# pierluigiferrari/ssd_keras

Hardware: AMD Instinct MI355X
Metric: images/sec SSD300 fwd+decode @batch32 (higher is better)
Workload: dtype f32 (decode, threshold, TF-style f32 NMS, top-k); bf16 conv backbone; 1 GPU; SSD300 VGG-16 inference (mode='inference': forward + DecodeDetections), 21 classes, batch 32 per GPU, conf 0.01 / NMS 0.45 / top-200, random-init weights, synthetic 300x300x3 uint8-range images; per_gpu_batch=32, global_batch=32, conv_dtype=bf16, parallelism=replicas x1, launch=hip_graph (forward + DecodeDetections captured once, replayed per step), decode_stream=same stream; DecodeDetections reads the head outputs directly (no y_pred in HBM)

## Files before the change

### ssd_keras_amd/csrc/ssdhip_decode.hip

```cpp
#include <hip/hip_runtime.h>
#include <stdint.h>
#include <stdlib.h>

#include "ssdhip.h"
#include "ssdhip_math.h"
#include "ssdhip_tile.h"
#include "ssdhip_heads.h"
#include "ssdhip_decode64.h"

#ifdef SSDHIP_PROFILE
__device__ unsigned long long g_prof[64];
#define PROF_DECL long long _pt = clock64(); long long _pa[12] = {0, 0, 0, 0, 0, 0, 0, 0, 0, 0, 0, 0};
#define PROF_MARK(i) { const long long _t = clock64(); _pa[i] += _t - _pt; _pt = _t; }
#define PROF_FLUSH(base) if (threadIdx.x == 0) { for (int _i = 0; _i < 12; ++_i) if (_pa[_i]) atomicAdd(&g_prof[(base) + _i], (unsigned long long)_pa[_i]); }
extern "C" int ssdhip_profile_read(unsigned long long* host_out, int reset) {
    if (hipMemcpyFromSymbol(host_out, HIP_SYMBOL(g_prof), sizeof(g_prof)) != hipSuccess) return -1;
    if (reset) { unsigned long long z[64] = {0}; if (hipMemcpyToSymbol(HIP_SYMBOL(g_prof), z, sizeof(z)) != hipSuccess) return -1; }
    return 0;
}
#else
#define PROF_DECL
#define PROF_MARK(i)
#define PROF_FLUSH(base)
#endif

namespace ssdhip {

constexpr int IDX_BITS = 20;
constexpr u32 IDX_MASK = (1u << IDX_BITS) - 1u;
constexpr int DIGIT_BITS = 13;
constexpr int NBINS = 1 << DIGIT_BITS;
constexpr int NMS_BIN_SHIFT = 14;
constexpr int NMS_NBINS = 4096;
#ifndef SSDHIP_MAX_CHUNK
#define SSDHIP_MAX_CHUNK 512
#endif
#ifndef SSDHIP_NMS_MINWAVES
#define SSDHIP_NMS_MINWAVES 3
#endif
constexpr int MAX_CHUNK = SSDHIP_MAX_CHUNK;
constexpr int KEPT_LDS = 256;
constexpr int KC_KEYS = 9216;
constexpr int TOPK_SORT_MAX = 4096;

struct DecodeParams {
    int B, N, C, L, G;
    int class_agnostic, semantics, coords, border;
    int thr_inclusive;
    float thr_eff;
    u32 thr_key;
    int iou_f32;
    int fast_ok;
    int px_f32;
    int no_nms;
    float filter_kE;
    double iou_thresh, img_w, img_h;
    int top_k, cap, cap_store, out_rows, sorted;
    int no_dma;
};

template <int SHIFT, int NB>
__device__ __forceinline__ int bin_of(u32 skey, u32 thr_key) {
    const u32 v = skey >> SHIFT, base = thr_key >> SHIFT;
    if (v <= base) return 0;
    const u32 d = v - base;
    return d > (u32)(NB - 1) ? NB - 1 : (int)d;
}

template <int SEM>
__device__ __forceinline__ float decode_center(float off, float var, float a_wh, float a_c) {
    if (SEM == SSDHIP_SEM_KERAS) return (off * var) * a_wh + a_c;
    if (SEM == SSDHIP_SEM_DEBUG) return (off * a_wh) * var + a_c;
    return off * (var * a_wh) + a_c;
}

__device__ __forceinline__ void scan_tile_body(const float* tile, int* wave_cnt, const DecodeParams& p, const int b, const int a0,
                                               const int na, float4* __restrict__ boxes, u64* __restrict__ cand,
                                               int* __restrict__ cand_count, unsigned short* __restrict__ cls_out) {
    const int TA = blockDim.x;
    const int L = p.L;
    const int tid = threadIdx.x;
    const int lane = tid & 63, wave = tid >> 6, nwaves = TA >> 6;
    PROF_DECL
    PROF_MARK(0)

    const bool active = tid < na;
    const float* row = tile + (size_t)tid * L;
    const int C = p.C;

    int fast_cls = 0;
    float fast_conf = 0.f;
    if (active) {
        const float o0 = row[C], o1 = row[C + 1], o2 = row[C + 2], o3 = row[C + 3];
        const float a_0 = row[C + 4], a_1 = row[C + 5], a_2 = row[C + 6], a_3 = row[C + 7];
        const float v0 = row[C + 8], v1 = row[C + 9], v2 = row[C + 10], v3 = row[C + 11];
        float4 box;
        if (p.coords == SSDHIP_CENTROIDS) {
            float cx, cy;
            if (p.semantics == SSDHIP_SEM_KERAS) {
                cx = decode_center<SSDHIP_SEM_KERAS>(o0, v0, a_2, a_0);
                cy = decode_center<SSDHIP_SEM_KERAS>(o1, v1, a_3, a_1);
            } else if (p.semantics == SSDHIP_SEM_DEBUG) {
                cx = decode_center<SSDHIP_SEM_DEBUG>(o0, v0, a_2, a_0);
                cy = decode_center<SSDHIP_SEM_DEBUG>(o1, v1, a_3, a_1);
            } else {
                cx = decode_center<SSDHIP_SEM_NUMPY>(o0, v0, a_2, a_0);
                cy = decode_center<SSDHIP_SEM_NUMPY>(o1, v1, a_3, a_1);
            }
            const float w = det_expf(o2 * v2) * a_2;
            const float h = det_expf(o3 * v3) * a_3;
            const float hw = w / 2.0f, hh = h / 2.0f;
            box = make_float4(cx - hw, cy - hh, cx + hw, cy + hh);
        } else if (p.coords == SSDHIP_MINMAX) {
            const float aw = a_1 - a_0, ah = a_3 - a_2;
            const float t0 = (o0 * v0) * aw + a_0, t1 = (o1 * v1) * aw + a_1;
            const float t2 = (o2 * v2) * ah + a_2, t3 = (o3 * v3) * ah + a_3;
            box = make_float4(t0, t2, t1, t3);
        } else {
            const float aw = a_2 - a_0, ah = a_3 - a_1;
            box = make_float4((o0 * v0) * aw + a_0, (o1 * v1) * ah + a_1, (o2 * v2) * aw + a_2, (o3 * v3) * ah + a_3);
        }
        boxes[(size_t)b * p.N + a0 + tid] = box;
        if (p.class_agnostic) {
            float best = row[0];
            int bi = 0;
            for (int c = 1; c < C; ++c) {
                const float s = row[c];
                if (s > best) { best = s; bi = c; }
            }
            for (int c = 0; c < C; ++c) if (row[c] != row[c]) { best = row[c]; bi = c; break; }
            fast_cls = bi;
            fast_conf = best;
            cls_out[(size_t)b * p.N + a0 + tid] = (unsigned short)bi;
        }
    }
    PROF_MARK(1)

    const int G = p.G;
    const float t = p.thr_eff;
    const bool incl = p.thr_inclusive != 0;
    const bool fast_pred = active && (fast_cls != 0) && (incl ? (fast_conf >= t) : (fast_conf > t));
    for (int gb = 0; gb < G; gb += 64) {
        const int ng = min(64, G - gb);
        int mycnt = 0;
        if (p.class_agnostic) {
            mycnt = __popcll(__ballot(fast_pred));
        } else {
            const float* sc = row + gb + 1;
            for (int j0 = 0; j0 < ng; j0 += 8) {
                float s8[8];
#pragma unroll
                for (int u = 0; u < 8; ++u) s8[u] = sc[min(j0 + u, ng - 1)];
#pragma unroll
                for (int u = 0; u < 8; ++u) {
                    const bool pr = active && (j0 + u < ng) && (incl ? (s8[u] >= t) : (s8[u] > t));
                    const int cnt = __popcll(__ballot(pr));
                    mycnt = lane == j0 + u ? cnt : mycnt;
                }
            }
        }
        if (lane < ng) wave_cnt[wave * G + gb + lane] = mycnt;
    }
    __syncthreads();
    PROF_MARK(2)
    for (int g = tid; g < G; g += TA) {
        int tot = 0;
        for (int w = 0; w < nwaves; ++w) tot += wave_cnt[w * G + g];
        int base = 0;
        if (tot) base = atomicAdd(&cand_count[b * G + g], tot);
        for (int w = 0; w < nwaves; ++w) {
            const int c = wave_cnt[w * G + g];
            wave_cnt[w * G + g] = base;
            base += c;
        }
    }
    __syncthreads();
    PROF_MARK(3)
    const u32 inv_idx = IDX_MASK - (u32)(a0 + tid);
    for (int gb = 0; gb < G; gb += 64) {
        const int ng = min(64, G - gb);
        const int mybase = lane < ng ? wave_cnt[wave * G + gb + lane] : 0;
        const float* sc = row + gb + 1;
        for (int j0 = 0; j0 < ng; j0 += 8) {
            float s8[8];
#pragma unroll
            for (int u = 0; u < 8; ++u) s8[u] = p.class_agnostic ? fast_conf : sc[min(j0 + u, ng - 1)];
#pragma unroll
            for (int u = 0; u < 8; ++u) {
                const int j = j0 + u;
                const float s = s8[u];
                const bool pr = (j < ng) && (p.class_agnostic ? fast_pred : (active && (incl ? (s >= t) : (s > t))));
                const u64 m = __ballot(pr);
                if (m == 0) continue;
                const int base_j = __builtin_amdgcn_readlane(mybase, j);
                if (pr) {
                    const int slot = base_j + (int)__builtin_amdgcn_mbcnt_hi((u32)(m >> 32), __builtin_amdgcn_mbcnt_lo((u32)m, 0u));
                    cand[((size_t)b * G + gb + j) * p.N + slot] = ((u64)float_key(s) << IDX_BITS) | inv_idx;
                }
            }
        }
    }
    PROF_MARK(4)
    PROF_FLUSH(16)
}

__global__ __launch_bounds__(256) void scan_kernel(const float* __restrict__ y, DecodeParams p,
                                                   float4* __restrict__ boxes, u64* __restrict__ cand,
                                                   int* __restrict__ cand_count, unsigned short* __restrict__ cls_out) {
    extern __shared__ __attribute__((aligned(16))) unsigned char smem_raw[];
    const int TA = blockDim.x;
    const int b = blockIdx.y;
    const int a0 = blockIdx.x * TA;
    const int na = min(TA, p.N - a0);
    const float* tile;
    const size_t total_bytes = (size_t)gridDim.y * p.N * (size_t)p.L * sizeof(float);
    if (!((uintptr_t)y & 15) && !(((size_t)p.N * p.L) & 3) && !((TA * p.L) & 3) && total_bytes < 0x7fffff00ull && !(TA & 63) && !p.no_dma) {
        const int lane = threadIdx.x & 63, wave = __builtin_amdgcn_readfirstlane((int)threadIdx.x >> 6);
        const u32 lds0 = (u32)(uintptr_t)(__attribute__((address_space(3))) unsigned char*)smem_raw;
        const i32x4 rs = tile_rsrc(y, (u32)total_bytes);
        const u32 off = (u32)(((size_t)b * p.N + a0) * (size_t)p.L * sizeof(float));
        const int nch = (na * p.L + 3) >> 2;
        for (int q0 = wave * 64; q0 < nch; q0 += TA) {
            const int q = q0 + lane;
            tile_dma16(q < nch ? off + (u32)q * 16u : TILE_OOB, rs, lds0 + (u32)q0 * 16u);
        }
        asm volatile("s_waitcnt vmcnt(0)" ::: "memory");
        tile = reinterpret_cast<const float*>(smem_raw);
    } else {
        tile = tile_copy_f32(reinterpret_cast<float*>(smem_raw), y + ((size_t)b * p.N + a0) * (size_t)p.L, na * p.L, threadIdx.x, TA);
    }
    int* wave_cnt = reinterpret_cast<int*>(smem_raw + (((size_t)TA * p.L + 4) * sizeof(float) + 15) / 16 * 16);
    __syncthreads();
    scan_tile_body(tile, wave_cnt, p, b, a0, na, boxes, cand, cand_count, cls_out);
}

constexpr int SW_WAVES = 4, SW_CW = 32, SW_PITCH = SW_CW + 1;
__global__ __launch_bounds__(SW_WAVES * 64) void scan_wide_kernel(const float* __restrict__ y, DecodeParams p, float4* __restrict__ boxes,
                                                                  u64* __restrict__ cand, int* __restrict__ cand_count) {
    __shared__ float win_all[SW_WAVES][64 * SW_PITCH];
    const int tid = threadIdx.x, lane = tid & 63, wave = tid >> 6;
    const int b = blockIdx.y;
    const int a0 = ((int)blockIdx.x * SW_WAVES + wave) * 64;
    if (a0 >= p.N) return;
    const int na = min(64, p.N - a0);
    float* win = win_all[wave];
    const int L = p.L, C = p.C, G = p.G;
    const float* src = y + ((size_t)b * p.N + a0) * (size_t)L;
    const float t = p.thr_eff;
    const bool incl = p.thr_inclusive != 0;
    const bool active = lane < na;
    const u32 inv_idx = IDX_MASK - (u32)(a0 + lane);
    const int nwin = (L + SW_CW - 1) / SW_CW;
    for (int wi = nwin - 1; wi >= 0; --wi) {
        const int c_hi = L - (nwin - 1 - wi) * SW_CW, c_lo = max(0, c_hi - SW_CW), cw = c_hi - c_lo;
        {
            const int c = lane & 31, rh = lane >> 5;
// ... 63 lines not shown
                if (m == 0) continue;
                const int base_j = __builtin_amdgcn_readlane(mybase, j);
                if (pr) {
                    const int slot = base_j + (int)__builtin_amdgcn_mbcnt_hi((u32)(m >> 32), __builtin_amdgcn_mbcnt_lo((u32)m, 0u));
                    cand[((size_t)b * G + (k_lo - 1) + j) * p.N + slot] = ((u64)float_key(sc) << IDX_BITS) | inv_idx;
                }
            }
        }
        __builtin_amdgcn_fence(__ATOMIC_ACQUIRE, "workgroup");
        __builtin_amdgcn_wave_barrier();
    }
}

__global__ __launch_bounds__(256) void scan_heads_kernel(HeadParams hp, const float* __restrict__ anchors_var, DecodeParams p,
                                                         float4* __restrict__ boxes, u64* __restrict__ cand,
                                                         int* __restrict__ cand_count, unsigned short* __restrict__ cls_out) {
    extern __shared__ __attribute__((aligned(16))) unsigned char smem_raw[];
    const int b = blockIdx.y;
    int l, a0, na;
    head_tile_of(hp, (int)blockIdx.x, l, a0, na);
    float* rows = reinterpret_cast<float*>(smem_raw);
    bf16_t* cl = reinterpret_cast<bf16_t*>(smem_raw + (size_t)hp.TA * p.L * sizeof(float));
    int* wave_cnt = reinterpret_cast<int*>(smem_raw + (head_tile_lds(hp.TA, p.C) + 15) / 16 * 16);
    head_build_rows(hp, anchors_var, l, b, a0, na, rows, cl, threadIdx.x, blockDim.x);
    scan_tile_body(rows, wave_cnt, p, b, hp.anchor_off[l] + a0, na, boxes, cand, cand_count, cls_out);
}

template <int KEY_BITS, int DB, int T, typename KeyF>
__device__ u64 block_select_kth(KeyF key_at, int n, u64 upper, bool has_upper, int k, u32* hist, int* red) {
    const int tid = threadIdx.x;
    constexpr int NB = 1 << DB;
    u64 prefix = 0, pmask = 0;
    constexpr int NPASS = (KEY_BITS + DB - 1) / DB;
    for (int pass = 0; pass < NPASS; ++pass) {
        const int shift = (NPASS - 1 - pass) * DB;
        for (int i = tid; i < NB; i += T) hist[i] = 0;
        __syncthreads();
        for (int i = tid; i < n; i += T) {
            const u64 key = key_at(i);
            if (has_upper && !(key < upper)) continue;
            if ((key & pmask) != prefix) continue;
            atomicAdd(&hist[(u32)(key >> shift) & (NB - 1)], 1u);
        }
        __syncthreads();
        block_find_digit<NB / T>(hist, k, red, red + 256);
        const int d = red[256];
        k -= red[257];
        prefix |= (u64)d << shift;
// ... 975 lines not shown
    if (p.px_f32 && ((double)(float)p.img_w != p.img_w || (double)(float)p.img_h != p.img_h)) return SSDHIP_E_BADARG;
    p.top_k = top_k; p.cap = nms_cap; p.cap_store = cap_store_for(N, top_k, nms_cap);
    p.out_rows = out_rows; p.sorted = sorted;

    unsigned char* base = static_cast<unsigned char*>(ws);
    float4* boxes = reinterpret_cast<float4*>(base + lay.boxes);
    int* cand_count = reinterpret_cast<int*>(base + lay.cand_count);
    int* kept_count = reinterpret_cast<int*>(base + lay.kept_count);
    unsigned short* cls_map = reinterpret_cast<unsigned short*>(base + lay.cls);
    u64* cand = reinterpret_cast<u64*>(base + lay.cand);
    u64* kept = reinterpret_cast<u64*>(base + lay.kept);

    if (stages & 1) {
    if (zero_async(cand_count, (size_t)B * p.G * sizeof(int), stream) != hipSuccess) return SSDHIP_E_LAUNCH;

    int TA = 256;
    while (TA > 64 && (size_t)TA * p.L * sizeof(float) > 24 * 1024) TA >>= 1;
    size_t k3_lds = align_up(((size_t)TA * p.L + 4) * sizeof(float), 16) + (size_t)(TA / 64) * p.G * sizeof(int);
    k3_lds = k3_lds > align_up((size_t)TA * p.L * sizeof(float), 1024) ? k3_lds : align_up((size_t)TA * p.L * sizeof(float), 1024);
    { const char* e = getenv("SSDHIP_SCAN_DMA"); p.no_dma = (e && e[0] == '0') ? 1 : 0; }
    if (k3_lds > 160 * 1024) return SSDHIP_E_BADARG;
    if (heads) {
        const int HT = heads->hp->TA;
        const size_t lds = (head_tile_lds(HT, C) + 15) / 16 * 16 + (size_t)((HT + 63) / 64) * p.G * sizeof(int);
        if (lds > 160 * 1024) return SSDHIP_E_BADARG;
        hipLaunchKernelGGL(scan_heads_kernel, dim3(heads->tiles, B), dim3(HT < 64 ? 64 : HT), lds, stream, *heads->hp,
                           heads->anchors_var, p, boxes, cand, cand_count, cls_map);
    } else if (p.L > 64 && !p.class_agnostic) {
        dim3 g3((N + SW_WAVES * 64 - 1) / (SW_WAVES * 64), B);
        hipLaunchKernelGGL(scan_wide_kernel, g3, dim3(SW_WAVES * 64), 0, stream, static_cast<const float*>(y_pred), p, boxes, cand, cand_count);
    } else {
        dim3 g3((N + TA - 1) / TA, B);
        hipLaunchKernelGGL(scan_kernel, g3, dim3(TA), k3_lds, stream, static_cast<const float*>(y_pred), p, boxes, cand,
                           cand_count, cls_map);
    }
    if (hipGetLastError() != hipSuccess) return SSDHIP_E_LAUNCH;
    }

    if (stages & 2) {
    const int work = B * p.G;
    const int g4 = ((work + 7) / 8) * 8;
    const int* order = nullptr;
    static const int nms_env = []() { const char* e = getenv("SSDHIP_NMS_T"); return e ? atoi(e) : 0; }();
    const int nms_t = nms_env ? nms_env : (semantics == SSDHIP_SEM_KERAS ? 512 : 256);
#define SSDHIP_LAUNCH_NMS(POL)                                                                                                            \
    do {                                                                                                                                  \
        if (nms_t >= 512) {                                                                                                               \
            hipLaunchKernelGGL((nms_kernel<POL, 512, false>), dim3(g4), dim3(512), 0, stream, p, boxes, cand, cand_count, order, kept, kept_count, 0); \
            hipLaunchKernelGGL((nms_kernel<POL, 512, true>), dim3(g4), dim3(512), 0, stream, p, boxes, cand, cand_count, order, kept, kept_count, 1); \
        } else {                                                                                                                          \
// ... 45 lines not shown
                                    void* ws, size_t ws_bytes, void* stream) {
    if (stages <= 0 || stages > 7) return SSDHIP_E_BADARG;
    return decode_run(nullptr, stages, y_pred, in_dtype, B, N, C, conf_thresh, iou_thresh, top_k, nms_cap, class_agnostic, semantics,
                      coords, normalize_coords, img_height, img_width, border_pixels, out, out_dtype, out_rows, out_count,
                      out_anchor_idx, ws, ws_bytes, stream);
}

static int decode_from_heads_any(int src_f32, int n_layers, const void* const* conf_h, const void* const* loc_h,
                                 const void* const* conf_bias_h, const void* const* loc_bias_h, const int* n_anchors_h,
                                 const int* n_boxes_h, const int* conf_stride_h, const int* loc_stride_h, const float* anchors_var,
                                 int B, int N, int C, double conf_thresh, double iou_thresh, int top_k, int nms_cap, int class_agnostic,
                                 int semantics, int coords, int normalize_coords, double img_height, double img_width, int border_pixels,
                                 void* out, int out_dtype, int out_rows, int* out_count, int* out_anchor_idx, void* ws, size_t ws_bytes,
                                 void* stream) {
    if (!anchors_var) return SSDHIP_E_BADARG;
    HeadParams hp;
    HeadSource src;
    src.hp = &hp; src.anchors_var = anchors_var; src.tiles = 0;
    size_t tile_lds = 60 * 1024;
#if defined(SSDHIP_PROFILE)
    if (const char* e = getenv("SSDHIP_HEADS_LDS_KB")) { const int v = atoi(e); if (v >= 8 && v <= 120) tile_lds = (size_t)v * 1024; }
#endif
    const int rc = head_fill_params(hp, n_layers, conf_h, loc_h, conf_bias_h, loc_bias_h, n_anchors_h, n_boxes_h, conf_stride_h,
                                    loc_stride_h, N, C, tile_lds, &src.tiles, src_f32);
    if (rc != SSDHIP_OK) return rc;
    if (hp.TA < 64) return SSDHIP_E_BADARG;
    return decode_run(&src, 7, nullptr, SSDHIP_F32, B, N, C, conf_thresh, iou_thresh, top_k, nms_cap, class_agnostic, semantics,
                      coords, normalize_coords, img_height, img_width, border_pixels, out, out_dtype, out_rows, out_count,
                      out_anchor_idx, ws, ws_bytes, stream);
}

extern "C" int ssdhip_decode_from_heads(int n_layers, const void* const* conf_h, const void* const* loc_h,
                                        const void* const* conf_bias_h, const void* const* loc_bias_h,
                                        const int* n_anchors_h, const int* n_boxes_h, const int* conf_stride_h,
                                        const int* loc_stride_h, const float* anchors_var, int B, int N, int C,
                                        double conf_thresh, double iou_thresh, int top_k, int nms_cap, int class_agnostic,
                                        int semantics, int coords, int normalize_coords, double img_height, double img_width,
                                        int border_pixels, void* out, int out_dtype, int out_rows, int* out_count,
                                        int* out_anchor_idx, void* ws, size_t ws_bytes, void* stream) {
    return decode_from_heads_any(0, n_layers, conf_h, loc_h, conf_bias_h, loc_bias_h, n_anchors_h, n_boxes_h, conf_stride_h, loc_stride_h,
                                 anchors_var, B, N, C, conf_thresh, iou_thresh, top_k, nms_cap, class_agnostic, semantics, coords,
                                 normalize_coords, img_height, img_width, border_pixels, out, out_dtype, out_rows, out_count,
                                 out_anchor_idx, ws, ws_bytes, stream);
}

extern "C" int ssdhip_decode_from_heads_f32(int n_layers, const void* const* conf_h, const void* const* loc_h, const int* n_anchors_h,
                                            const int* n_boxes_h, const int* conf_stride_h, const int* loc_stride_h,
// ... 10 lines not shown
```

### ssd_keras_amd/csrc/ssdhip_heads.h

```cpp
#pragma once
#include <hip/hip_runtime.h>
#include <stdint.h>
#include <stdlib.h>

#include "ssdhip.h"
#include "ssdhip_math.h"
#include "ssdhip_bf16.h"
#include "ssdhip_tile.h"

namespace ssdhip {

constexpr int MAX_PRED_LAYERS = 8;
struct HeadParams {
    const bf16_t* conf[MAX_PRED_LAYERS];
    const bf16_t* loc[MAX_PRED_LAYERS];
    const bf16_t* conf_bias[MAX_PRED_LAYERS];
    const bf16_t* loc_bias[MAX_PRED_LAYERS];
    int n_anchors[MAX_PRED_LAYERS];
    int n_boxes[MAX_PRED_LAYERS];
    int conf_stride[MAX_PRED_LAYERS];
    int loc_stride[MAX_PRED_LAYERS];
    int tile_start[MAX_PRED_LAYERS + 1];
    int anchor_off[MAX_PRED_LAYERS];
    int n_layers, N, C, TA;
    int row_dma;
    int src_f32;
};

__host__ __device__ inline size_t head_stage_bytes(int TA, int C) {
    return (size_t)TA * (C + 4) * sizeof(bf16_t) + (size_t)16 * TA + (size_t)64 * (C + 4) + 1024;
}
__host__ __device__ inline size_t head_tile_lds(int TA, int C) { return (size_t)TA * (C + 12) * sizeof(float) + head_stage_bytes(TA, C); }

__device__ __forceinline__ void head_tile_of(const HeadParams& hp, int tile_id, int& l, int& a0, int& na) {
    l = 0;
    while (l + 1 < hp.n_layers && tile_id >= hp.tile_start[l + 1]) ++l;
    a0 = (tile_id - hp.tile_start[l]) * hp.TA;
    na = min(hp.TA, hp.n_anchors[l] - a0);
}

__device__ __forceinline__ void head_build_rows(const HeadParams& hp, const float* __restrict__ anchors_var, int l, int b, int a0, int na,
                                                float* rows, bf16_t* cl, int tid, int nthreads) {
    const int TA = hp.TA, C = hp.C, L = C + 12;
    bf16_t* ll = cl + (size_t)TA * C;
    const int nb = hp.n_boxes[l];
    if (hp.src_f32) {
        const size_t px0 = (size_t)b * (hp.n_anchors[l] / nb);
        {
            const int step_a = nthreads / C, step_c = nthreads - step_a * C;
            int c = tid % C, a = tid / C;
            const int ga0 = a0 + a;
            int pix = ga0 / nb, box = ga0 - pix * nb;
            const float* src = reinterpret_cast<const float*>(hp.conf[l]) + px0 * hp.conf_stride[l];
            const int cs = hp.conf_stride[l];
            const int q0 = step_a / nb, r0 = step_a - q0 * nb, q1 = (step_a + 1) / nb, r1 = step_a + 1 - q1 * nb;
            for (int i = tid; i < na * C; i += nthreads) {
                rows[(size_t)a * L + c] = src[(size_t)pix * cs + box * C + c];
                c += step_c;
                const bool carry = c >= C;
                c -= carry ? C : 0;
                a += step_a + (carry ? 1 : 0);
                box += carry ? r1 : r0;
                pix += carry ? q1 : q0;
                if (box >= nb) { box -= nb; ++pix; }
            }
// ... 10 lines not shown
            for (int i = tid; i < na * 4; i += nthreads) {
                rows[(size_t)a * L + C + k] = src[(size_t)pix * ls + box * 4 + k];
                a += step_a;
                box += r0;
                pix += q0;
                if (box >= nb) { box -= nb; ++pix; }
            }
        }
        __syncthreads();
        for (int a = tid; a < na; a += nthreads) {
            float* r = rows + (size_t)a * L;
            float mx = -INFINITY;
            for (int c = 0; c < C; ++c) mx = fmaxf(mx, r[c]);
            float sum = 0.f;
            for (int c = 0; c < C; ++c) { const float e = expf(r[c] - mx); r[c] = e; sum += e; }
            for (int c = 0; c < C; ++c) r[c] = r[c] / sum;
            const float* av = anchors_var + (size_t)(hp.anchor_off[l] + a0 + a) * 8;
            for (int k = 0; k < 8; ++k) r[C + 4 + k] = av[k];
        }
        __syncthreads();
        return;
    }
    {
        const int stride = hp.conf_stride[l];
        const int U = nb * (C + 4) * 2, cpr = (U + 15) >> 4, pitch = cpr * 16;
        const int pix0 = a0 / nb, npx = (a0 + na - 1) / nb - pix0 + 1, nchunks = npx * cpr;
        const size_t dma_area = (size_t)((nchunks + 63) >> 6) * 1024;
        const size_t npix_l = (size_t)(hp.n_anchors[l] / nb);
        const size_t src_bytes = (size_t)gridDim.y * npix_l * (size_t)stride * 2;
        const bool dma = hp.row_dma && hp.loc[l] == hp.conf[l] + (size_t)nb * C && hp.loc_stride[l] == stride && !(stride & 7) && stride * 2 >= pitch &&
                         !((uintptr_t)hp.conf[l] & 15) && dma_area + (size_t)U <= head_stage_bytes(TA, C) && src_bytes < 0x7fffff00ull &&
                         !(nthreads & 63);
        if (dma) {
            unsigned char* st = reinterpret_cast<unsigned char*>(cl);
            const u32 lds0 = (u32)(uintptr_t)(__attribute__((address_space(3))) unsigned char*)st;
            const i32x4 rs = tile_rsrc(hp.conf[l], (u32)src_bytes);
            const int lane = tid & 63, wave = __builtin_amdgcn_readfirstlane(tid >> 6);
            const u32 row0 = (u32)(((size_t)b * npix_l + pix0) * (size_t)stride * 2);
            for (int q0 = wave * 64; q0 < nchunks; q0 += nthreads) {
                const int q = q0 + lane, r = q / cpr, j = q - r * cpr;
                tile_dma16(q < nchunks ? row0 + (u32)r * (u32)(stride * 2) + (u32)j * 16u : TILE_OOB, rs, lds0 + (u32)q0 * 16u);
            }
            bf16_t* bs = reinterpret_cast<bf16_t*>(st + dma_area);
            const bool has_cb = hp.conf_bias[l] != nullptr, has_lb = hp.loc_bias[l] != nullptr;
            if (has_cb) for (int i = tid; i < nb * C; i += nthreads) bs[i] = hp.conf_bias[l][i];
            if (has_lb) for (int i = tid; i < nb * 4; i += nthreads) bs[nb * C + i] = hp.loc_bias[l][i];
            const bool av16 = !((uintptr_t)anchors_var & 15);
            float4 av0 = make_float4(0.f, 0.f, 0.f, 0.f), av1 = av0;
            if (av16 && tid < na) {
                const float4* avp = reinterpret_cast<const float4*>(anchors_var + (size_t)(hp.anchor_off[l] + a0 + tid) * 8);
                av0 = avp[0]; av1 = avp[1];
            }
            asm volatile("s_waitcnt vmcnt(0)" ::: "memory");
            __syncthreads();
            for (int a = tid; a < na; a += nthreads) {
                const int ga = a0 + a, pix = ga / nb, box = ga - pix * nb;
                const bf16_t* prow = reinterpret_cast<const bf16_t*>(st + (size_t)(pix - pix0) * pitch);
                const bf16_t* src = prow + box * C;
                const bf16_t* cb = bs + box * C;
                float* r = rows + (size_t)a * L;
                float mx = -INFINITY;
                int c = 0;
                for (; c + 4 <= C; c += 4) {
                    float v[4];
#pragma unroll
                    for (int u = 0; u < 4; ++u) {
                        const float x = bf16_float(src[c + u]);
                        v[u] = has_cb ? bf16_float(bf16_bits(x + bf16_float(cb[c + u]))) : x;
                    }
#pragma unroll
                    for (int u = 0; u < 4; ++u) { r[c + u] = v[u]; mx = fmaxf(mx, v[u]); }
                }
                for (; c < C; ++c) {
                    const float x = bf16_float(src[c]);
                    const float v = has_cb ? bf16_float(bf16_bits(x + bf16_float(cb[c]))) : x;
                    r[c] = v;
                    mx = fmaxf(mx, v);
                }
                float sum = 0.f;
                for (c = 0; c + 4 <= C; c += 4) {
                    float e[4];
#pragma unroll
                    for (int u = 0; u < 4; ++u) e[u] = r[c + u];
#pragma unroll
                    for (int u = 0; u < 4; ++u) { e[u] = expf(e[u] - mx); sum += e[u]; }
#pragma unroll
                    for (int u = 0; u < 4; ++u) r[c + u] = e[u];
                }
                for (; c < C; ++c) { const float e = expf(r[c] - mx); r[c] = e; sum += e; }
                for (c = 0; c + 4 <= C; c += 4) {
                    float e[4];
#pragma unroll
                    for (int u = 0; u < 4; ++u) e[u] = r[c + u];
#pragma unroll
                    for (int u = 0; u < 4; ++u) r[c + u] = e[u] / sum;
                }
                for (; c < C; ++c) r[c] = r[c] / sum;
                const bf16_t* lsrc = prow + nb * C + box * 4;
                const bf16_t* lb = bs + nb * C + box * 4;
#pragma unroll
                for (int k = 0; k < 4; ++k) r[C + k] = has_lb ? bf16_float(bf16_bits(bf16_float(lsrc[k]) + bf16_float(lb[k]))) : bf16_float(lsrc[k]);
                if (av16 && a == tid) {
                    r[C + 4] = av0.x; r[C + 5] = av0.y; r[C + 6] = av0.z; r[C + 7] = av0.w;
                    r[C + 8] = av1.x; r[C + 9] = av1.y; r[C + 10] = av1.z; r[C + 11] = av1.w;
                } else {
                    const float* av = anchors_var + (size_t)(hp.anchor_off[l] + a0 + a) * 8;
                    for (int k = 0; k < 8; ++k) r[C + 4 + k] = av[k];
                }
            }
            __syncthreads();
            return;
        }
    }
    if (hp.conf_stride[l] == nb * C && hp.loc_stride[l] == nb * 4) {
        const bf16_t* csrc = hp.conf[l] + ((size_t)b * hp.n_anchors[l] + a0) * C;
        const bf16_t* lsrc = hp.loc[l] + ((size_t)b * hp.n_anchors[l] + a0) * 4;
        for (int i = tid; i < na * C; i += nthreads) cl[i] = csrc[i];
        for (int i = tid; i < na * 4; i += nthreads) ll[i] = lsrc[i];
    } else {
        const size_t px0 = (size_t)b * (hp.n_anchors[l] / nb);
        {
            const int step_a = nthreads / C, step_c = nthreads - step_a * C;
            int c = tid % C;
            const int ga0 = a0 + tid / C;
            int pix = ga0 / nb, box = ga0 - pix * nb;
            const bf16_t* src = hp.conf[l] + px0 * hp.conf_stride[l];
            const int cs = hp.conf_stride[l];
            const int q0 = step_a / nb, r0 = step_a - q0 * nb, q1 = (step_a + 1) / nb, r1 = step_a + 1 - q1 * nb;
            for (int i = tid; i < na * C; i += nthreads) {
                cl[i] = src[(size_t)pix * cs + box * C + c];
                c += step_c;
                const bool carry = c >= C;
                c -= carry ? C : 0;
// ... 23 lines not shown
        const int box = (a0 + a) % nb;
        float* r = rows + (size_t)a * L;
        const bf16_t* cb = hp.conf_bias[l] ? hp.conf_bias[l] + box * C : nullptr;
        float mx = -INFINITY;
        for (int c = 0; c < C; ++c) {
            const float v = cb ? bf16_float(bf16_bits(bf16_float(cl[a * C + c]) + bf16_float(cb[c]))) : bf16_float(cl[a * C + c]);
            r[c] = v;
            mx = fmaxf(mx, v);
        }
        float sum = 0.f;
        for (int c = 0; c < C; ++c) { const float e = expf(r[c] - mx); r[c] = e; sum += e; }
        for (int c = 0; c < C; ++c) r[c] = r[c] / sum;
        const bf16_t* lb = hp.loc_bias[l] ? hp.loc_bias[l] + box * 4 : nullptr;
        for (int k = 0; k < 4; ++k) r[C + k] = lb ? bf16_float(bf16_bits(bf16_float(ll[a * 4 + k]) + bf16_float(lb[k]))) : bf16_float(ll[a * 4 + k]);
        const float* av = anchors_var + (size_t)(hp.anchor_off[l] + a0 + a) * 8;
        for (int k = 0; k < 8; ++k) r[C + 4 + k] = av[k];
    }
    __syncthreads();
}

static inline int head_fill_params(HeadParams& hp, int n_layers, const void* const* conf_h, const void* const* loc_h,
                                   const void* const* conf_bias_h, const void* const* loc_bias_h, const int* n_anchors_h,
                                   const int* n_boxes_h, const int* conf_stride_h, const int* loc_stride_h, int N, int C,
                                   size_t max_lds, int* tiles_out, int src_f32 = 0) {
    if (n_layers <= 0 || n_layers > MAX_PRED_LAYERS || !conf_h || !loc_h || !n_anchors_h || !n_boxes_h || N <= 0 || C < 2 || C > 1024)
        return SSDHIP_E_BADARG;
    int TA = 256;
    while (TA > 32 && head_tile_lds(TA, C) > max_lds) TA >>= 1;
    hp.n_layers = n_layers; hp.N = N; hp.C = C; hp.TA = TA; hp.src_f32 = src_f32 ? 1 : 0;
    { const char* e = getenv("SSDHIP_HEADS_DMA"); hp.row_dma = !(e && e[0] == '0'); }
    if (src_f32 && (conf_bias_h || loc_bias_h)) {
        for (int l = 0; l < n_layers; ++l)
            if ((conf_bias_h && conf_bias_h[l]) || (loc_bias_h && loc_bias_h[l])) return SSDHIP_E_BADARG;
    }
    int off = 0, tiles = 0;
    for (int l = 0; l < MAX_PRED_LAYERS; ++l) {
        const bool on = l < n_layers;
        hp.conf[l] = on ? static_cast<const bf16_t*>(conf_h[l]) : nullptr;
        hp.loc[l] = on ? static_cast<const bf16_t*>(loc_h[l]) : nullptr;
        hp.conf_bias[l] = (on && conf_bias_h) ? static_cast<const bf16_t*>(conf_bias_h[l]) : nullptr;
        hp.loc_bias[l] = (on && loc_bias_h) ? static_cast<const bf16_t*>(loc_bias_h[l]) : nullptr;
        hp.n_anchors[l] = on ? n_anchors_h[l] : 0;
        hp.n_boxes[l] = on ? n_boxes_h[l] : 1;
        hp.conf_stride[l] = on ? (conf_stride_h ? conf_stride_h[l] : n_boxes_h[l] * C) : 0;
        hp.loc_stride[l] = on ? (loc_stride_h ? loc_stride_h[l] : n_boxes_h[l] * 4) : 0;
        hp.tile_start[l] = tiles;
        hp.anchor_off[l] = off;
        if (on) {
            if (!hp.conf[l] || !hp.loc[l] || hp.n_anchors[l] <= 0 || hp.n_boxes[l] <= 0 || hp.n_anchors[l] % hp.n_boxes[l]) return SSDHIP_E_BADARG;
            if (hp.conf_stride[l] < hp.n_boxes[l] * C || hp.loc_stride[l] < hp.n_boxes[l] * 4) return SSDHIP_E_BADARG;
            off += hp.n_anchors[l];
            tiles += (hp.n_anchors[l] + TA - 1) / TA;
        }
    }
    hp.tile_start[MAX_PRED_LAYERS] = tiles;
    if (off != N) return SSDHIP_E_BADARG;
    *tiles_out = tiles;
    return SSDHIP_OK;
}

}
```

Before: 16910 images/sec.

## Keep per-anchor softmax scores in registers for fused head scan kernel

Adds a register-resident scan path for the fused head decode. Each thread builds its anchor's softmax scores and box/anchor values in a fixed-size register array instead of writing float rows to LDS. The scan body is templated over the row source so LDS and register forms share one body. It is enabled by default when C<=32 and every tile qualifies for the DMA staging path, and it fixes the tile width at 256 with a launch-bounds occupancy hint. The aim is to cut LDS footprint and LDS traffic so more blocks fit per CU, at the cost of higher register pressure from fully unrolled per-class loops. Profiling hooks for the head build phases are also added.

```diff
diff --git a/ssd_keras_amd/csrc/ssdhip_decode.hip b/ssd_keras_amd/csrc/ssdhip_decode.hip
--- a/ssd_keras_amd/csrc/ssdhip_decode.hip
+++ b/ssd_keras_amd/csrc/ssdhip_decode.hip
@@ -13,6 +13,9 @@
 #define PROF_DECL long long _pt = clock64(); long long _pa[12] = {0, 0, 0, 0, 0, 0, 0, 0, 0, 0, 0, 0};
 #define PROF_MARK(i) { const long long _t = clock64(); _pa[i] += _t - _pt; _pt = _t; }
 #define PROF_FLUSH(base) if (threadIdx.x == 0) { for (int _i = 0; _i < 12; ++_i) if (_pa[_i]) atomicAdd(&g_prof[(base) + _i], (unsigned long long)_pa[_i]); }
+#define HEADS_PROF_DECL long long _hp[5] = {0, 0, 0, 0, 0};
+#define HEADS_PROF_ARG , _hp
+#define HEADS_PROF_FLUSH if (threadIdx.x == 0) { for (int _i = 0; _i < 5; ++_i) atomicAdd(&g_prof[21 + _i], (unsigned long long)_hp[_i]); }
 extern "C" int ssdhip_profile_read(unsigned long long* host_out, int reset) {
     if (hipMemcpyFromSymbol(host_out, HIP_SYMBOL(g_prof), sizeof(g_prof)) != hipSuccess) return -1;
     if (reset) { unsigned long long z[64] = {0}; if (hipMemcpyToSymbol(HIP_SYMBOL(g_prof), z, sizeof(z)) != hipSuccess) return -1; }
@@ -22,6 +25,9 @@
 #define PROF_DECL
 #define PROF_MARK(i)
 #define PROF_FLUSH(base)
+#define HEADS_PROF_DECL
+#define HEADS_PROF_ARG
+#define HEADS_PROF_FLUSH
 #endif
 
 namespace ssdhip {
@@ -37,6 +43,9 @@
 #endif
 #ifndef SSDHIP_NMS_MINWAVES
 #define SSDHIP_NMS_MINWAVES 3
+#endif
+#ifndef SSDHIP_SCAN_REG_MINWAVES
+#define SSDHIP_SCAN_REG_MINWAVES 5
 #endif
 constexpr int MAX_CHUNK = SSDHIP_MAX_CHUNK;
 constexpr int KEPT_LDS = 256;
@@ -74,26 +83,65 @@
     return off * (var * a_wh) + a_c;
 }
 
-__device__ __forceinline__ void scan_tile_body(const float* tile, int* wave_cnt, const DecodeParams& p, const int b, const int a0,
+struct LdsRow {
+    const float* row;
+    int C;
+    __device__ __forceinline__ float box(int k) const { return row[C + k]; }
+    template <typename F>
+    __device__ __forceinline__ void each_score(int c0, int n, F&& f) const {
+        for (int j = 0; j < n; ++j) f(j, row[c0 + j]);
+    }
+    template <typename F>
+    __device__ __forceinline__ void each_score8(int c0, int n, F&& f) const {
+        const float* sc = row + c0;
+        for (int j0 = 0; j0 < n; j0 += 8) {
+            float s8[8];
+#pragma unroll
+            for (int u = 0; u < 8; ++u) s8[u] = sc[min(j0 + u, n - 1)];
+#pragma unroll
+            for (int u = 0; u < 8; ++u) f(j0 + u, s8[u], j0 + u < n);
+        }
+    }
+};
+
+template <int CMAX>
+struct RegRow {
+    float v[CMAX];
+    float bx[12];
+    __device__ __forceinline__ float box(int k) const { return bx[k]; }
+    template <typename F>
+    __device__ __forceinline__ void each_score(int c0, int n, F&& f) const {
+#pragma unroll
+        for (int c = 0; c < CMAX; ++c)
+            if (c >= c0 && c - c0 < n) f(c - c0, v[c]);
+    }
+    template <typename F>
+    __device__ __forceinline__ void each_score8(int c0, int n, F&& f) const {
+#pragma unroll
+        for (int c = 0; c < CMAX; ++c)
+            if (c >= c0 && c - c0 < n) f(c - c0, v[c], true);
+    }
+};
+
+template <typename Row>
+__device__ __forceinline__ void scan_tile_body(const Row& row, int* wave_cnt, const DecodeParams& p, const int b, const int a0,
                                                const int na, float4* __restrict__ boxes, u64* __restrict__ cand,
                                                int* __restrict__ cand_count, unsigned short* __restrict__ cls_out) {
     const int TA = blockDim.x;
-    const int L = p.L;
     const int tid = threadIdx.x;
     const int lane = tid & 63, wave = tid >> 6, nwaves = TA >> 6;
     PROF_DECL
     PROF_MARK(0)
 
     const bool active = tid < na;
-    const float* row = tile + (size_t)tid * L;
     const int C = p.C;
 
     int fast_cls = 0;
     float fast_conf = 0.f;
     if (active) {
-        const float o0 = row[C], o1 = row[C + 1], o2 = row[C + 2], o3 = row[C + 3];
-        const float a_0 = row[C + 4], a_1 = row[C + 5], a_2 = row[C + 6], a_3 = row[C + 7];
-        const float v0 = row[C + 8], v1 = row[C + 9], v2 = row[C + 10], v3 = row[C + 11];
+        const float o0 = row.box(0), o1 = row.box(1), o2 = row.box(2), o3 = row.box(3);
+        const float a_0 = row.box(4), a_1 = row.box(5), a_2 = row.box(6), a_3 = row.box(7);
+        const float v0 = row.box(8), v1 = row.box(9), v2 = row.box(10), v3 = row.box(11);
         float4 box;
         if (p.coords == SSDHIP_CENTROIDS) {
             float cx, cy;
@@ -122,13 +170,15 @@
         }
         boxes[(size_t)b * p.N + a0 + tid] = box;
         if (p.class_agnostic) {
-            float best = row[0];
+            float best = 0.f;
             int bi = 0;
-            for (int c = 1; c < C; ++c) {
-                const float s = row[c];
-                if (s > best) { best = s; bi = c; }
-            }
-            for (int c = 0; c < C; ++c) if (row[c] != row[c]) { best = row[c]; bi = c; break; }
+            row.each_score(0, C, [&](int c, float s) {
+                if (c == 0 || s > best) { best = s; bi = c; }
+            });
+            bool has_nan = false;
+            row.each_score(0, C, [&](int c, float s) {
+                if (!has_nan && s != s) { best = s; bi = c; has_nan = true; }
+            });
             fast_cls = bi;
             fast_conf = best;
             cls_out[(size_t)b * p.N + a0 + tid] = (unsigned short)bi;
@@ -146,18 +196,11 @@
         if (p.class_agnostic) {
             mycnt = __popcll(__ballot(fast_pred));
         } else {
-            const float* sc = row + gb + 1;
-            for (int j0 = 0; j0 < ng; j0 += 8) {
-                float s8[8];
-#pragma unroll
-                for (int u = 0; u < 8; ++u) s8[u] = sc[min(j0 + u, ng - 1)];
-#pragma unroll
-                for (int u = 0; u < 8; ++u) {
-                    const bool pr = active && (j0 + u < ng) && (incl ? (s8[u] >= t) : (s8[u] > t));
-                    const int cnt = __popcll(__ballot(pr));
-                    mycnt = lane == j0 + u ? cnt : mycnt;
-                }
-            }
+            row.each_score8(gb + 1, ng, [&](int j, float s, bool valid) {
+                const bool pr = active && valid && (incl ? (s >= t) : (s > t));
+                const int cnt = __popcll(__ballot(pr));
+                mycnt = lane == j ? cnt : mycnt;
+            });
         }
         if (lane < ng) wave_cnt[wave * G + gb + lane] = mycnt;
     }
@@ -180,24 +223,21 @@
     for (int gb = 0; gb < G; gb += 64) {
         const int ng = min(64, G - gb);
         const int mybase = lane < ng ? wave_cnt[wave * G + gb + lane] : 0;
-        const float* sc = row + gb + 1;
-        for (int j0 = 0; j0 < ng; j0 += 8) {
-            float s8[8];
-#pragma unroll
-            for (int u = 0; u < 8; ++u) s8[u] = p.class_agnostic ? fast_conf : sc[min(j0 + u, ng - 1)];
-#pragma unroll
-            for (int u = 0; u < 8; ++u) {
-                const int j = j0 + u;
-                const float s = s8[u];
-                const bool pr = (j < ng) && (p.class_agnostic ? fast_pred : (active && (incl ? (s >= t) : (s > t))));
-                const u64 m = __ballot(pr);
-                if (m == 0) continue;
-                const int base_j = __builtin_amdgcn_readlane(mybase, j);
-                if (pr) {
-                    const int slot = base_j + (int)__builtin_amdgcn_mbcnt_hi((u32)(m >> 32), __builtin_amdgcn_mbcnt_lo((u32)m, 0u));
-                    cand[((size_t)b * G + gb + j) * p.N + slot] = ((u64)float_key(s) << IDX_BITS) | inv_idx;
-                }
-            }
+        const auto emit = [&](int j, float s, bool pr) {
+            const u64 m = __ballot(pr);
+            if (m == 0) return;
+            const int base_j = __builtin_amdgcn_readlane(mybase, j);
+            if (pr) {
+                const int slot = base_j + (int)__builtin_amdgcn_mbcnt_hi((u32)(m >> 32), __builtin_amdgcn_mbcnt_lo((u32)m, 0u));
+                cand[((size_t)b * G + gb + j) * p.N + slot] = ((u64)float_key(s) << IDX_BITS) | inv_idx;
+            }
+        };
+        if (p.class_agnostic) {
+            emit(0, fast_conf, fast_pred);
+        } else {
+            row.each_score8(gb + 1, ng, [&](int j, float s, bool valid) {
+                emit(j, s, active && valid && (incl ? (s >= t) : (s > t)));
+            });
         }
     }
     PROF_MARK(4)
@@ -231,7 +271,7 @@
     }
     int* wave_cnt = reinterpret_cast<int*>(smem_raw + (((size_t)TA * p.L + 4) * sizeof(float) + 15) / 16 * 16);
     __syncthreads();
-    scan_tile_body(tile, wave_cnt, p, b, a0, na, boxes, cand, cand_count, cls_out);
+    scan_tile_body(LdsRow{tile + (size_t)threadIdx.x * p.L, p.C}, wave_cnt, p, b, a0, na, boxes, cand, cand_count, cls_out);
 }
 
 constexpr int SW_WAVES = 4, SW_CW = 32, SW_PITCH = SW_CW + 1;
@@ -341,8 +381,27 @@
     float* rows = reinterpret_cast<float*>(smem_raw);
     bf16_t* cl = reinterpret_cast<bf16_t*>(smem_raw + (size_t)hp.TA * p.L * sizeof(float));
     int* wave_cnt = reinterpret_cast<int*>(smem_raw + (head_tile_lds(hp.TA, p.C) + 15) / 16 * 16);
-    head_build_rows(hp, anchors_var, l, b, a0, na, rows, cl, threadIdx.x, blockDim.x);
-    scan_tile_body(rows, wave_cnt, p, b, hp.anchor_off[l] + a0, na, boxes, cand, cand_count, cls_out);
+    HEADS_PROF_DECL
+    head_build_rows(hp, anchors_var, l, b, a0, na, rows, cl, threadIdx.x, blockDim.x HEADS_PROF_ARG);
+    HEADS_PROF_FLUSH
+    scan_tile_body(LdsRow{rows + (size_t)threadIdx.x * p.L, p.C}, wave_cnt, p, b, hp.anchor_off[l] + a0, na, boxes, cand, cand_count, cls_out);
+}
+
+template <int CMAX>
+__global__ __launch_bounds__(256, SSDHIP_SCAN_REG_MINWAVES) void scan_heads_reg_kernel(HeadParams hp, const float* __restrict__ anchors_var,
+                                                                                       DecodeParams p, float4* __restrict__ boxes,
+                                                                                       u64* __restrict__ cand, int* __restrict__ cand_count,
+                                                                                       unsigned short* __restrict__ cls_out) {
+    extern __shared__ __attribute__((aligned(16))) unsigned char smem_raw[];
+    const int b = blockIdx.y;
+    int l, a0, na;
+    head_tile_of(hp, (int)blockIdx.x, l, a0, na);
+    int* wave_cnt = reinterpret_cast<int*>(smem_raw + (head_stage_bytes(hp.TA, p.C) + 15) / 16 * 16);
+    RegRow<CMAX> row;
+    HEADS_PROF_DECL
+    head_build_regs(hp, anchors_var, l, b, a0, na, smem_raw, threadIdx.x, blockDim.x, row.v, row.bx HEADS_PROF_ARG);
+    HEADS_PROF_FLUSH
+    scan_tile_body(row, wave_cnt, p, b, hp.anchor_off[l] + a0, na, boxes, cand, cand_count, cls_out);
 }
 
 template <int KEY_BITS, int DB, int T, typename KeyF>
@@ -1364,10 +1423,21 @@
     if (k3_lds > 160 * 1024) return SSDHIP_E_BADARG;
     if (heads) {
         const int HT = heads->hp->TA;
-        const size_t lds = (head_tile_lds(HT, C) + 15) / 16 * 16 + (size_t)((HT + 63) / 64) * p.G * sizeof(int);
-        if (lds > 160 * 1024) return SSDHIP_E_BADARG;
-        hipLaunchKernelGGL(scan_heads_kernel, dim3(heads->tiles, B), dim3(HT < 64 ? 64 : HT), lds, stream, *heads->hp,
-                           heads->anchors_var, p, boxes, cand, cand_count, cls_map);
+        const size_t cnt_lds = (size_t)((HT + 63) / 64) * p.G * sizeof(int);
+        if (heads->hp->reg_form) {
+            const size_t lds = (head_stage_bytes(HT, C) + 15) / 16 * 16 + cnt_lds;
+            if (C <= HEAD_REG_CSMALL)
+                hipLaunchKernelGGL(scan_heads_reg_kernel<HEAD_REG_CSMALL>, dim3(heads->tiles, B), dim3(HT), lds, stream, *heads->hp,
+                                   heads->anchors_var, p, boxes, cand, cand_count, cls_map);
+            else
+                hipLaunchKernelGGL(scan_heads_reg_kernel<HEAD_REG_CMAX>, dim3(heads->tiles, B), dim3(HT), lds, stream, *heads->hp,
+                                   heads->anchors_var, p, boxes, cand, cand_count, cls_map);
+        } else {
+            const size_t lds = (head_tile_lds(HT, C) + 15) / 16 * 16 + cnt_lds;
+            if (lds > 160 * 1024) return SSDHIP_E_BADARG;
+            hipLaunchKernelGGL(scan_heads_kernel, dim3(heads->tiles, B), dim3(HT < 64 ? 64 : HT), lds, stream, *heads->hp,
+                               heads->anchors_var, p, boxes, cand, cand_count, cls_map);
+        }
     } else if (p.L > 64 && !p.class_agnostic) {
         dim3 g3((N + SW_WAVES * 64 - 1) / (SW_WAVES * 64), B);
         hipLaunchKernelGGL(scan_wide_kernel, g3, dim3(SW_WAVES * 64), 0, stream, static_cast<const float*>(y_pred), p, boxes, cand, cand_count);
@@ -1459,7 +1529,7 @@
     if (const char* e = getenv("SSDHIP_HEADS_LDS_KB")) { const int v = atoi(e); if (v >= 8 && v <= 120) tile_lds = (size_t)v * 1024; }
 #endif
     const int rc = head_fill_params(hp, n_layers, conf_h, loc_h, conf_bias_h, loc_bias_h, n_anchors_h, n_boxes_h, conf_stride_h,
-                                    loc_stride_h, N, C, tile_lds, &src.tiles, src_f32);
+                                    loc_stride_h, N, C, tile_lds, &src.tiles, src_f32, B);
     if (rc != SSDHIP_OK) return rc;
     if (hp.TA < 64) return SSDHIP_E_BADARG;
     return decode_run(&src, 7, nullptr, SSDHIP_F32, B, N, C, conf_thresh, iou_thresh, top_k, nms_cap, class_agnostic, semantics,
diff --git a/ssd_keras_amd/csrc/ssdhip_heads.h b/ssd_keras_amd/csrc/ssdhip_heads.h
--- a/ssd_keras_amd/csrc/ssdhip_heads.h
+++ b/ssd_keras_amd/csrc/ssdhip_heads.h
@@ -25,7 +25,19 @@
     int n_layers, N, C, TA;
     int row_dma;
     int src_f32;
+    int reg_form;
 };
+
+constexpr int HEAD_REG_CMAX = 32;
+constexpr int HEAD_REG_CSMALL = 24;
+
+#ifdef SSDHIP_PROFILE
+#define HEAD_PROF_DECL long long _hpt = clock64();
+#define HEAD_PROF_MARK(i) { const long long _t = clock64(); if (prof) prof[i] += _t - _hpt; _hpt = _t; }
+#else
+#define HEAD_PROF_DECL
+#define HEAD_PROF_MARK(i)
+#endif
 
 __host__ __device__ inline size_t head_stage_bytes(int TA, int C) {
     return (size_t)TA * (C + 4) * sizeof(bf16_t) + (size_t)16 * TA + (size_t)64 * (C + 4) + 1024;
@@ -39,8 +51,109 @@
     na = min(hp.TA, hp.n_anchors[l] - a0);
 }
 
+__host__ __device__ inline bool head_tile_dma_ok(const HeadParams& hp, int l, int a0, int na, int B, int nthreads) {
+    const int nb = hp.n_boxes[l], C = hp.C, stride = hp.conf_stride[l];
+    const int U = nb * (C + 4) * 2, cpr = (U + 15) >> 4, pitch = cpr * 16;
+    const int pix0 = a0 / nb, npx = (a0 + na - 1) / nb - pix0 + 1, nchunks = npx * cpr;
+    const size_t dma_area = (size_t)((nchunks + 63) >> 6) * 1024;
+    const size_t src_bytes = (size_t)B * (size_t)(hp.n_anchors[l] / nb) * (size_t)stride * 2;
+    return hp.row_dma && !hp.src_f32 && hp.loc[l] == hp.conf[l] + (size_t)nb * C && hp.loc_stride[l] == stride && !(stride & 7) && stride * 2 >= pitch &&
+           !((uintptr_t)hp.conf[l] & 15) && dma_area + (size_t)U <= head_stage_bytes(hp.TA, C) && src_bytes < 0x7fffff00ull && !(nthreads & 63);
+}
+
+struct HeadStage {
+    int pitch, pix0;
+    const bf16_t* bs;
+    bool has_cb, has_lb;
+};
+
+__device__ __forceinline__ HeadStage head_stage_issue(const HeadParams& hp, int l, int b, int a0, int na, unsigned char* st, int tid, int nthreads) {
+    const int C = hp.C, nb = hp.n_boxes[l], stride = hp.conf_stride[l];
+    const int U = nb * (C + 4) * 2, cpr = (U + 15) >> 4, pitch = cpr * 16;
+    const int pix0 = a0 / nb, npx = (a0 + na - 1) / nb - pix0 + 1, nchunks = npx * cpr;
+    const size_t dma_area = (size_t)((nchunks + 63) >> 6) * 1024;
+    const size_t npix_l = (size_t)(hp.n_anchors[l] / nb);
+    const size_t src_bytes = (size_t)gridDim.y * npix_l * (size_t)stride * 2;
+    const u32 lds0 = (u32)(uintptr_t)(__attribute__((address_space(3))) unsigned char*)st;
+    const i32x4 rs = tile_rsrc(hp.conf[l], (u32)src_bytes);
+    const int lane = tid & 63, wave = __builtin_amdgcn_readfirstlane(tid >> 6);
+    const u32 row0 = (u32)(((size_t)b * npix_l + pix0) * (size_t)stride * 2);
+    for (int q0 = wave * 64; q0 < nchunks; q0 += nthreads) {
+        const int q = q0 + lane, r = q / cpr, j = q - r * cpr;
+        tile_dma16(q < nchunks ? row0 + (u32)r * (u32)(stride * 2) + (u32)j * 16u : TILE_OOB, rs, lds0 + (u32)q0 * 16u);
+    }
+    bf16_t* bs = reinterpret_cast<bf16_t*>(st + dma_area);
+    HeadStage hs;
+    hs.pitch = pitch; hs.pix0 = pix0; hs.bs = bs;
+    hs.has_cb = hp.conf_bias[l] != nullptr; hs.has_lb = hp.loc_bias[l] != nullptr;
+    if (hs.has_cb) for (int i = tid; i < nb * C; i += nthreads) bs[i] = hp.conf_bias[l][i];
+    if (hs.has_lb) for (int i = tid; i < nb * 4; i += nthreads) bs[nb * C + i] = hp.loc_bias[l][i];
+    return hs;
+}
+
+__device__ __forceinline__ float head_biased(bf16_t x, bool has_bias, const bf16_t* bias) {
+    return has_bias ? bf16_float(bf16_bits(bf16_float(x) + bf16_float(*bias))) : bf16_float(x);
+}
+
+template <int CMAX>
+__device__ __forceinline__ void head_build_regs(const HeadParams& hp, const float* __restrict__ anchors_var, int l, int b, int a0, int na,
+                                                unsigned char* st, int tid, int nthreads, float (&v)[CMAX], float (&bx)[12],
+                                                long long* prof = nullptr) {
+    HEAD_PROF_DECL
+    const int C = hp.C, nb = hp.n_boxes[l];
+    const HeadStage hs = head_stage_issue(hp, l, b, a0, na, st, tid, nthreads);
+    const bool active = tid < na;
+#pragma unroll
+    for (int c = 0; c < CMAX; ++c) v[c] = 0.f;
+#pragma unroll
+    for (int k = 0; k < 12; ++k) bx[k] = 0.f;
+    if (active) {
+        const float* av = anchors_var + (size_t)(hp.anchor_off[l] + a0 + tid) * 8;
+        if (!((uintptr_t)anchors_var & 15)) {
+            const float4 av0 = reinterpret_cast<const float4*>(av)[0], av1 = reinterpret_cast<const float4*>(av)[1];
+            bx[4] = av0.x; bx[5] = av0.y; bx[6] = av0.z; bx[7] = av0.w;
+            bx[8] = av1.x; bx[9] = av1.y; bx[10] = av1.z; bx[11] = av1.w;
+        } else {
+#pragma unroll
+            for (int k = 0; k < 8; ++k) bx[4 + k] = av[k];
+        }
+    }
+    asm volatile("s_waitcnt vmcnt(0)" ::: "memory");
+    __syncthreads();
+    HEAD_PROF_MARK(0)
+    if (active) {
+        const int ga = a0 + tid, pix = ga / nb, box = ga - pix * nb;
+        const bf16_t* prow = reinterpret_cast<const bf16_t*>(st + (size_t)(pix - hs.pix0) * hs.pitch);
+        const bf16_t* src = prow + box * C;
+        const bf16_t* cb = hs.bs + box * C;
+        float mx = -INFINITY;
+#pragma unroll
+        for (int c = 0; c < CMAX; ++c)
+            if (c < C) v[c] = head_biased(src[c], hs.has_cb, cb + c);
+#pragma unroll
+        for (int c = 0; c < CMAX; ++c)
+            if (c < C) mx = fmaxf(mx, v[c]);
+        HEAD_PROF_MARK(1)
+        float sum = 0.f;
+#pragma unroll
+        for (int c = 0; c < CMAX; ++c)
+            if (c < C) { v[c] = expf(v[c] - mx); sum += v[c]; }
+        HEAD_PROF_MARK(2)
+#pragma unroll
+        for (int c = 0; c < CMAX; ++c)
+            if (c < C) v[c] = v[c] / sum;
+        HEAD_PROF_MARK(3)
+        const bf16_t* lsrc = prow + nb * C + box * 4;
+        const bf16_t* lb = hs.bs + nb * C + box * 4;
+#pragma unroll
+        for (int k = 0; k < 4; ++k) bx[k] = head_biased(lsrc[k], hs.has_lb, lb + k);
+    }
+    HEAD_PROF_MARK(4)
+}
+
 __device__ __forceinline__ void head_build_rows(const HeadParams& hp, const float* __restrict__ anchors_var, int l, int b, int a0, int na,
-                                                float* rows, bf16_t* cl, int tid, int nthreads) {
+                                                float* rows, bf16_t* cl, int tid, int nthreads, long long* prof = nullptr) {
+    HEAD_PROF_DECL
     const int TA = hp.TA, C = hp.C, L = C + 12;
     bf16_t* ll = cl + (size_t)TA * C;
     const int nb = hp.n_boxes[l];
@@ -97,29 +210,12 @@
         return;
     }
     {
-        const int stride = hp.conf_stride[l];
-        const int U = nb * (C + 4) * 2, cpr = (U + 15) >> 4, pitch = cpr * 16;
-        const int pix0 = a0 / nb, npx = (a0 + na - 1) / nb - pix0 + 1, nchunks = npx * cpr;
-        const size_t dma_area = (size_t)((nchunks + 63) >> 6) * 1024;
-        const size_t npix_l = (size_t)(hp.n_anchors[l] / nb);
-        const size_t src_bytes = (size_t)gridDim.y * npix_l * (size_t)stride * 2;
-        const bool dma = hp.row_dma && hp.loc[l] == hp.conf[l] + (size_t)nb * C && hp.loc_stride[l] == stride && !(stride & 7) && stride * 2 >= pitch &&
-                         !((uintptr_t)hp.conf[l] & 15) && dma_area + (size_t)U <= head_stage_bytes(TA, C) && src_bytes < 0x7fffff00ull &&
-                         !(nthreads & 63);
-        if (dma) {
+        if (head_tile_dma_ok(hp, l, a0, na, (int)gridDim.y, nthreads)) {
             unsigned char* st = reinterpret_cast<unsigned char*>(cl);
-            const u32 lds0 = (u32)(uintptr_t)(__attribute__((address_space(3))) unsigned char*)st;
-            const i32x4 rs = tile_rsrc(hp.conf[l], (u32)src_bytes);
-            const int lane = tid & 63, wave = __builtin_amdgcn_readfirstlane(tid >> 6);
-            const u32 row0 = (u32)(((size_t)b * npix_l + pix0) * (size_t)stride * 2);
-            for (int q0 = wave * 64; q0 < nchunks; q0 += nthreads) {
-                const int q = q0 + lane, r = q / cpr, j = q - r * cpr;
-                tile_dma16(q < nchunks ? row0 + (u32)r * (u32)(stride * 2) + (u32)j * 16u : TILE_OOB, rs, lds0 + (u32)q0 * 16u);
-            }
-            bf16_t* bs = reinterpret_cast<bf16_t*>(st + dma_area);
-            const bool has_cb = hp.conf_bias[l] != nullptr, has_lb = hp.loc_bias[l] != nullptr;
-            if (has_cb) for (int i = tid; i < nb * C; i += nthreads) bs[i] = hp.conf_bias[l][i];
-            if (has_lb) for (int i = tid; i < nb * 4; i += nthreads) bs[nb * C + i] = hp.loc_bias[l][i];
+            const HeadStage hs = head_stage_issue(hp, l, b, a0, na, st, tid, nthreads);
+            const int pitch = hs.pitch, pix0 = hs.pix0;
+            const bf16_t* bs = hs.bs;
+            const bool has_cb = hs.has_cb, has_lb = hs.has_lb;
             const bool av16 = !((uintptr_t)anchors_var & 15);
             float4 av0 = make_float4(0.f, 0.f, 0.f, 0.f), av1 = av0;
             if (av16 && tid < na) {
@@ -128,6 +224,7 @@
             }
             asm volatile("s_waitcnt vmcnt(0)" ::: "memory");
             __syncthreads();
+            HEAD_PROF_MARK(0)
             for (int a = tid; a < na; a += nthreads) {
                 const int ga = a0 + a, pix = ga / nb, box = ga - pix * nb;
                 const bf16_t* prow = reinterpret_cast<const bf16_t*>(st + (size_t)(pix - pix0) * pitch);
@@ -152,6 +249,7 @@
                     r[c] = v;
                     mx = fmaxf(mx, v);
                 }
+                HEAD_PROF_MARK(1)
                 float sum = 0.f;
                 for (c = 0; c + 4 <= C; c += 4) {
                     float e[4];
@@ -163,6 +261,7 @@
                     for (int u = 0; u < 4; ++u) r[c + u] = e[u];
                 }
                 for (; c < C; ++c) { const float e = expf(r[c] - mx); r[c] = e; sum += e; }
+                HEAD_PROF_MARK(2)
                 for (c = 0; c + 4 <= C; c += 4) {
                     float e[4];
 #pragma unroll
@@ -171,6 +270,7 @@
                     for (int u = 0; u < 4; ++u) r[c + u] = e[u] / sum;
                 }
                 for (; c < C; ++c) r[c] = r[c] / sum;
+                HEAD_PROF_MARK(3)
                 const bf16_t* lsrc = prow + nb * C + box * 4;
                 const bf16_t* lb = bs + nb * C + box * 4;
 #pragma unroll
@@ -184,6 +284,7 @@
                 }
             }
             __syncthreads();
+            HEAD_PROF_MARK(4)
             return;
         }
     }
@@ -253,7 +354,7 @@
 static inline int head_fill_params(HeadParams& hp, int n_layers, const void* const* conf_h, const void* const* loc_h,
                                    const void* const* conf_bias_h, const void* const* loc_bias_h, const int* n_anchors_h,
                                    const int* n_boxes_h, const int* conf_stride_h, const int* loc_stride_h, int N, int C,
-                                   size_t max_lds, int* tiles_out, int src_f32 = 0) {
+                                   size_t max_lds, int* tiles_out, int src_f32 = 0, int reg_B = 0) {
     if (n_layers <= 0 || n_layers > MAX_PRED_LAYERS || !conf_h || !loc_h || !n_anchors_h || !n_boxes_h || N <= 0 || C < 2 || C > 1024)
         return SSDHIP_E_BADARG;
     int TA = 256;
@@ -286,6 +387,26 @@
     }
     hp.tile_start[MAX_PRED_LAYERS] = tiles;
     if (off != N) return SSDHIP_E_BADARG;
+    hp.reg_form = 0;
+    const char* reg_env = getenv("SSDHIP_HEADS_REG");
+    if (reg_B > 0 && !src_f32 && C <= HEAD_REG_CMAX && !(reg_env && reg_env[0] == '0')) {
+        constexpr int TR = 256;
+        hp.TA = TR;
+        bool ok = true;
+        for (int l = 0; l < n_layers && ok; ++l)
+            for (int a0 = 0; a0 < hp.n_anchors[l] && ok; a0 += TR) ok = head_tile_dma_ok(hp, l, a0, hp.n_anchors[l] - a0 < TR ? hp.n_anchors[l] - a0 : TR, reg_B, TR);
+        if (ok) {
+            hp.reg_form = 1;
+            tiles = 0;
+            for (int l = 0; l < MAX_PRED_LAYERS; ++l) {
+                hp.tile_start[l] = tiles;
+                if (l < n_layers) tiles += (hp.n_anchors[l] + TR - 1) / TR;
+            }
+            hp.tile_start[MAX_PRED_LAYERS] = tiles;
+        } else {
+            hp.TA = TA;
+        }
+    }
     *tiles_out = tiles;
     return SSDHIP_OK;
 }
```

After: 17040 images/sec, median of 6. About the same (+0.7%).
